# cbrl/BNN-PYNQ

Measured on AMD Instinct MI355X. Metric: images/sec (whole node) CNV-W1A1 CIFAR-10-shape batch, higher is better.
Workload: dtype u1; 1 GPU; cnvW1A1, 131072 synthetic 32x32x3 uint8 images per GPU per step, inputs resident in HBM, params cifar10/cnvW1A1; parallelism=dp1 (batch shards, no data-path collective)

## Files before the change

### bnn-pynq_amd/csrc/kernels.hip

```cpp
#include <hip/hip_runtime.h>
#include <hip/hip_ext.h>
#include <stdint.h>

#include <cstdlib>
#include <cstring>
#include <type_traits>

#define BNN_HD __host__ __device__
#include "act_faults.h"
#include "input_faults.h"
#include "kernels.h"
#include "mem_faults.h"
#include "mem_org.h"
#include "packed_params.h"
static_assert(bnn::kL0TileOffset == (int)bnn::kL0MfmaTileOffset && bnn::kL0BigBytes == (int)bnn::kL0MfmaBigBytes,
              "k_conv0_tile's operand offsets must be the ones packed_params.cpp writes the layer-0 table by");

namespace bnn {
namespace {

typedef const uint32_t __attribute__((address_space(4))) *kptr32;
typedef const uint64_t __attribute__((address_space(4))) *kptr64;

constexpr int kBlock = 256;
// ... 704 lines not shown
    for (int t0 = (wave / NT) * 32; t0 < nitems; t0 += 32 * STREAMS) {
      const int item = min(t0 + c, nitems - 1);
      const int i = item / IPI, rem = item - i * IPI, rp = rem / WOUT, x = rem - rp * WOUT;
      v16f acc[2] = {seed, seed};
#pragma unroll
      for (int kh = 0; kh < KH; kh++) {
        const uint4 *__restrict__ P = &plane[i][kh * 2 + h][2 * rp * WIN + x];
#pragma unroll
        for (int kx = 0; kx < 3; kx++) {
          v8i b[4];
#pragma unroll
          for (int y = 0; y < 4; y++) {
            const uint4 v = P[y * WIN + kx];
            b[y] = v8i{(int)v.x, (int)v.y, (int)v.z, (int)v.w, 0, 0, 0, 0};
          }
#pragma unroll
          for (int ky = 0; ky < 3; ky++)
#pragma unroll
            for (int dy = 0; dy < 2; dy++)
              acc[dy] = __builtin_amdgcn_mfma_scale_f32_32x32x64_f8f6f4(wreg[(ky * 3 + kx) * KH + kh], b[ky + dy], acc[dy], 4, 4, 0,
                                                                         0x7F7F7F7F, 0, 0x7F7F7F7F);
        }
      }
      const bool valid = t0 + c < nitems;
      const size_t img = (size_t)(img0 + i);
      if constexpr (POOL) {
        v16f top;
#pragma unroll
        for (int k = 0; k < 16; k++) top[k] = fmaxf(acc[0][k], acc[1][k]);
        uint32_t n0, n1;
        not_fired(top, dt, h, n0, n1);
        n0 &= (uint32_t)__builtin_amdgcn_mov_dpp((int)n0, 0xB1, 0xF, 0xF, true);
        n1 &= (uint32_t)__builtin_amdgcn_mov_dpp((int)n1, 0xB1, 0xF, 0xF, true);
        const size_t w64 = (img * (RP * RP) + rp * RP + (x >> 1)) * (NT / 2) + mt / 2;
        if (valid && !(x & 1)) out[(w64 * 2 + h) * 2 + (mt & 1)] = h ? ~(n0 ^ n1) : (n0 & n1);
      } else {
        uint32_t n0[2], n1[2];
#pragma unroll
        for (int dy = 0; dy < 2; dy++) not_fired(acc[dy], dt, h, n0[dy], n1[dy]);
        const uint32_t m0 = h ? n0[1] : n0[0], m1 = h ? n1[1] : n1[0];
        const size_t w64 = (img * (WOUT * WOUT) + (2 * rp + h) * WOUT + x) * (NT / 2) + mt / 2;
        if (valid) {
          out[(w64 * 2 + 0) * 2 + (mt & 1)] = m0 & m1;
          out[(w64 * 2 + 1) * 2 + (mt & 1)] = ~(m0 ^ m1);
        }
      }
    }
  }
}

template <bool TT>
__global__ __launch_bounds__(256) void k_conv_mfma_a2_table(const uint32_t *__restrict__ rows, int ksteps, int tiles,
                                                             uint8_t *__restrict__ dst) {
  const int idx = blockIdx.x * 256 + threadIdx.x, nw = ksteps * tiles * 64, row_dw = TT ? 4 + 6 * ksteps : 2 + 2 * ksteps;
  if (idx < nw) {
    const int ks = idx / (tiles * 64), mt = (idx / 64) % tiles, lane = idx & 63, n = 32 * mt + (lane & 31), h = lane >> 5;
    const uint32_t *__restrict__ row = rows + (size_t)n * row_dw;
    uint32_t b1, b2 = 0, b3;
    if constexpr (TT) {
      const uint32_t sg = row[2 + 4 * ks + h], two = row[2 + 4 * ksteps + 2 * ks + h], nz = row[2 + 4 * ks + 2 + h] | two;
      b1 = nz & ~two;
      b2 = two;
      b3 = (sg & nz) | two;
    } else {
      b1 = 0xFFFFFFFFu;
      b3 = row[2 + 2 * ks + h];
    }
    uint32_t v[4];
#pragma unroll
    for (int k = 0; k < 4; k++)
      v[k] = (nibble_spread(b1 >> (8 * k)) << 1) | (nibble_spread(b2 >> (8 * k)) << 2) | (nibble_spread(b3 >> (8 * k)) << 3);
    reinterpret_cast<uint4 *>(dst)[idx] = make_uint4(v[0], v[1], v[2], v[3]);
  } else if (idx < nw + tiles * 64) {
    const int j = idx - nw, second = j >= tiles * 32, jj = second ? j - tiles * 32 : j, mt = jj >> 5, h = (jj >> 4) & 1, reg = jj & 15;
    const int n = 32 * mt + (reg & 3) + 8 * (reg >> 2) + 4 * h;
    const int lim = 2 * 64 * ksteps;
    int t0 = (int)rows[(size_t)n * row_dw], t1 = (int)rows[(size_t)n * row_dw + 1];
    t0 = t0 < -lim - 1 ? -lim - 1 : (t0 > lim ? lim : t0);
    t1 = t1 < -lim - 1 ? -lim - 1 : (t1 > lim ? lim : t1);
    reinterpret_cast<float *>(dst + (size_t)nw * 16)[j] = second ? (float)(t1 - t0) : -(float)t0 - 0.5f;
  }
}

template <bool A2, int KS, int NT, bool CONV, int WAVES, int G>
__global__ __launch_bounds__(64 * WAVES, 8 / WAVES) void k_tail_mfma(const std::conditional_t<A2, uint4, uint32_t> *__restrict__ in,
                                                                      uint32_t *__restrict__ out, const uint8_t *__restrict__ tab,
                                                                      int n_images) {
  using U = std::conditional_t<A2, uint4, uint32_t>;
  constexpr int T = 64 * WAVES, TPW = NT / WAVES, IPI = CONV ? 9 : 1, W64 = CONV ? 25 * 2 : KS, UPI = A2 ? W64 : 2 * W64;
  constexpr int GP = G + 1, NPL = CONV ? G * 4 * 25 : 2 * KS * GP, NPF = (G * UPI + T - 1) / T, NC = (A2 ? 2 : 1) * NT * 2;
  static_assert(NT % WAVES == 0 && (!CONV || KS == 18) && (G * IPI) % 32 == 0, "tile geometry");
  __shared__ uint4 plane[NPL];
  __shared__ uint32_t lut[A2 ? 512 : 256];
  __shared__ v16f cst[NC];
  const int tid = threadIdx.x, lane = tid & 63, wave = tid >> 6, mt0 = wave * TPW, c = lane & 31, h = lane >> 5;
  for (int k = tid; k < 256; k += T) {
    if constexpr (A2) {
      lut[k] = nibble_spread((uint32_t)k) << 1;
      lut[256 + k] = nibble_spread((uint32_t)k) << 3;
    } else {
      lut[k] = fp4_pm1((uint32_t)k);
    }
  }
  for (int k = tid; k < NC * 16; k += T) reinterpret_cast<float *>(cst)[k] = reinterpret_cast<const float *>(tab + (size_t)KS * NT * 64 * 16)[k];
  const uint4 *__restrict__ wt = reinterpret_cast<const uint4 *>(tab);
  v8i wreg[TPW][KS];
#pragma unroll
  for (int j = 0; j < TPW; j++)
#pragma unroll
    for (int ks = 0; ks < KS; ks++) {
      const uint4 v = wt[(ks * NT + mt0 + j) * 64 + lane];
      wreg[j][ks] = v8i{(int)v.x, (int)v.y, (int)v.z, (int)v.w, 0, 0, 0, 0};
    }
  const int ngroups = (n_images + G - 1) / G;
  U pre[NPF];
  auto fetch = [&](int grp) {
    const int img0 = grp * G, lim = min(G, n_images - img0) * UPI;
#pragma unroll
    for (int j = 0; j < NPF; j++) {
      const int d = tid + T * j;
      pre[j] = d < lim ? in[(size_t)img0 * UPI + d] : U{};
    }
  };
  if (blockIdx.x < ngroups) fetch(blockIdx.x);
  for (int grp = blockIdx.x; grp < ngroups; grp += gridDim.x) {
    const int img0 = grp * G, nimg = min(G, n_images - img0), nitems = nimg * IPI;
    __syncthreads();
#pragma unroll
    for (int j = 0; j < NPF; j++) {
      const int d = tid + T * j;
      if (d < nimg * UPI) {
        const int i = d / UPI, e = d - i * UPI;
        if constexpr (A2) {
          const uint4 v = pre[j];
          const int p0 = CONV ? (i * 4 + 2 * (e & 1)) * 25 + (e >> 1) : 2 * e * GP + i, step = CONV ? 25 : GP;
          plane[p0] = fp4_planes(lut, lut + 256, v.x, v.z);
          plane[p0 + step] = fp4_planes(lut, lut + 256, v.y, v.w);
        } else {
          const uint32_t bits = pre[j];
          const int p0 = CONV ? (i * 4 + (e & 3)) * 25 + (e >> 2) : e * GP + i;
          plane[p0] = make_uint4(lut[bits & 255], lut[(bits >> 8) & 255], lut[(bits >> 16) & 255], lut[bits >> 24]);
        }
      }
    }
    if (grp + (int)gridDim.x < ngroups) fetch(grp + gridDim.x);
    __syncthreads();
#pragma clang loop unroll(disable) interleave(disable) vectorize(disable)
    for (int t0 = 0; t0 < nitems; t0 += 32) {
      const int item = min(t0 + c, nitems - 1);
      int base;
      if constexpr (CONV) {
        const int i = item / 9, p = item - i * 9, oy = p / 3, ox = p - oy * 3;
        base = (i * 4 + h) * 25 + oy * 5 + ox;
      } else {
        base = h * GP + item;
      }
      v16f acc[TPW];
#pragma unroll
      for (int j = 0; j < TPW; j++) acc[j] = cst[(mt0 + j) * 2 + h];
#pragma unroll
      for (int ks = 0; ks < KS; ks++) {
        const int off = CONV ? (ks & 1) * 2 * 25 + ((ks >> 1) / 3) * 5 + (ks >> 1) % 3 : ks * 2 * GP;
        const uint4 v = plane[base + off];
        const v8i b = v8i{(int)v.x, (int)v.y, (int)v.z, (int)v.w, 0, 0, 0, 0};
#pragma unroll
        for (int j = 0; j < TPW; j++)
          acc[j] = __builtin_amdgcn_mfma_scale_f32_32x32x64_f8f6f4(wreg[j][ks], b, acc[j], 4, 4, 0, 0x7F7F7F7F, 0, 0x7F7F7F7F);
      }
      const bool valid = t0 + c < nitems;
      const size_t gitem = (size_t)img0 * IPI + item;
#pragma unroll
      for (int j = 0; j < TPW; j++) {
        const int mt = mt0 + j;
        if constexpr (A2) {
          uint32_t n0, n1;
          not_fired(acc[j], cst[NT * 2 + mt * 2 + h], h, n0, n1);
          const size_t w64 = gitem * (NT / 2) + mt / 2;
          if (valid) out[(w64 * 2 + h) * 2 + (mt & 1)] = h ? ~(n0 ^ n1) : (n0 & n1);
        } else {
          int v[16];
#pragma unroll
          for (int k = 0; k < 16; k++) v[k] = __float_as_int(acc[j][k]);
          const uint32_t nf = or_halves(sign_nibbles(v, h));
          if (valid && h == (j & 1)) out[gitem * NT + mt] = ~nf;
        }
      }
    }
  }
}

__device__ __forceinline__ uint32_t chain_temp() {
  uint32_t t;
  asm("" : "=v"(t));
  return t;
}
#ifdef BNN_VGPR_COUNTER
#define SCALAR_COUNTER(c) do { } while (0)
#else
#define SCALAR_COUNTER(c) asm volatile("" : "+s"(c))
#endif
__device__ __forceinline__ void xpop(int &acc, uint32_t w, uint32_t a, uint32_t &t) {
  asm("v_xor_b32 %0, %2, %3\n\tv_bcnt_u32_b32 %1, %0, %1" : "+v"(t), "+v"(acc) : "s"(w), "v"(a));
}
__device__ __forceinline__ void xpop4(int &m0, int &m1, int &m2, int &m3, uint32_t w, uint32_t a0, uint32_t a1,
                                      uint32_t a2, uint32_t a3, uint32_t &t) {
  xpop(m0, w, a0, t); xpop(m1, w, a1, t); xpop(m2, w, a2, t); xpop(m3, w, a3, t);
}
__device__ __forceinline__ int xpop_seed(uint32_t w, uint32_t a, int seed, uint32_t &t) {
  int acc;
  asm("v_xor_b32 %0, %2, %3\n\tv_bcnt_u32_b32 %1, %0, %4" : "+v"(t), "=v"(acc) : "s"(w), "v"(a), "s"(seed));
  return acc;
}
template <int NPB>
__device__ __forceinline__ void store_group(uint32_t *__restrict__ out, size_t index, uint32_t bits) {
  if constexpr (NPB == 32) out[index] = bits;
  else reinterpret_cast<uint8_t *>(out)[index] = (uint8_t)bits;
}

template <int CW, int ID, bool POOL, int NPB = 32, bool MULTI = false>
__global__ __launch_bounds__(kBlock) void k_quad_x(const uint64_t *__restrict__ in, uint32_t *__restrict__ out,
                                                    const uint32_t *__restrict__ rows, int n_items, int groups, int gpb, MultiArgs ma = {}) {
  constexpr int OD = ID - 2, QD = OD / 2, NQ = QD * QD, KW = 9 * CW, ROW_DW = 2 + 2 * KW;
  int item0 = 0;
  if constexpr (MULTI) item0 = multi_prologue(ma, rows, out, n_items, 0);
  const BlockMap bm = map_block(groups / gpb, n_items);
  if (!bm.valid) return;
  const int item = bm.item + item0;
  const int img = item / NQ, q = item - img * NQ;
  const int qy = q / QD, qx = q - qy * QD;
  const uint64_t *__restrict__ base = in + ((size_t)img * ID * ID + (size_t)(2 * qy) * ID + 2 * qx) * CW;
  uint32_t wl[4][4][CW], wh[4][4][CW];
#pragma unroll
  for (int y = 0; y < 4; y++)
#pragma unroll
    for (int x = 0; x < 4; x++)
#pragma unroll
      for (int k = 0; k < CW; k++) {
        const uint64_t v = base[(y * ID + x) * CW + k];
        wl[y][x][k] = (uint32_t)v;
        wh[y][x][k] = (uint32_t)(v >> 32);
      }
  uint32_t t = chain_temp();
  for (int cg = bm.cg * gpb, cg_end = cg + gpb; cg < cg_end; cg++) {
    kptr32 w = (kptr32)(uintptr_t)(rows + (size_t)cg * NPB * ROW_DW);
    uint32_t b[4] = {0, 0, 0, 0};
    for (int c = NPB - 1; c >= 0; c--) {
      kptr32 r = w + c * ROW_DW;
      SCALAR_COUNTER(c);
      const int nt = -(int)r[0];
      int m[2][2];
  #pragma unroll
      for (int j = 0; j < KW; j++) {
        const int ky = j / (3 * CW), kx = (j / CW) % 3, k = j % CW;
        const uint32_t w0 = r[2 + 2 * j], w1 = r[3 + 2 * j];
        if (j == 0) {
  #pragma unroll
          for (int i = 0; i < 4; i++) m[i >> 1][i & 1] = xpop_seed(w0, wl[ky + (i >> 1)][kx + (i & 1)][k], nt, t);
        } else {
          xpop4(m[0][0], m[0][1], m[1][0], m[1][1], w0, wl[ky][kx][k], wl[ky][kx + 1][k], wl[ky + 1][kx][k], wl[ky + 1][kx + 1][k], t);
        }
        xpop4(m[0][0], m[0][1], m[1][0], m[1][1], w1, wh[ky][kx][k], wh[ky][kx + 1][k], wh[ky + 1][kx][k], wh[ky + 1][kx + 1][k], t);
      }
      if constexpr (POOL) {
        b[0] = shift_in_sign(b[0], min(min(m[0][0], m[0][1]), min(m[1][0], m[1][1])));
      } else {
  #pragma unroll
        for (int i = 0; i < 4; i++) b[i] = shift_in_sign(b[i], m[i >> 1][i & 1]);
      }
    }
// ... 502 lines not shown
  constexpr bool TWO = ARITH == AR_TT;
  constexpr int KW = 9 * CW, ROW_DW = row_dw<ARITH, KW>(), OD = ID - 2, NPIX = POOL ? (OD / 2) * (OD / 2) : OD * OD;
  const MultiSeg sg = multi_seg(ma);
  const int item0 = multi_prologue(ma, rows, out, n_items, 0);
  const BlockMap bm = map_block(groups / gpb, n_items);
  if (!bm.valid) return;
  const ActWinSite st = win_site(sites, sg.run);
  const WinItem wi = win_item<ID, POOL>(bm.item + item0, sg, st.y, st.x);
  const uint64_t *__restrict__ in = base + ((size_t)wi.image * ID * ID + (size_t)wi.oy * ID + wi.ox) * CW * 2;
  uint32_t as[KW][2], az[KW][2];
#pragma unroll
  for (int ky = 0; ky < 3; ky++)
#pragma unroll
    for (int kx = 0; kx < 3; kx++) {
      const bool hit = wi.oy + ky == st.y && wi.ox + kx == st.x;
#pragma unroll
      for (int k = 0; k < CW; k++) {
        const uint64_t *__restrict__ src = in + ((ky * ID + kx) * CW + k) * 2;
        uint64_t sgn = src[0], nz = src[1];
        if (hit && k == st.word) {
          const uint64_t m = 1ull << st.bit;
          const uint32_t i = (sgn & m) ? 0u : ((nz & m) ? 2u : 1u), lv = (i + (uint32_t)st.shift) % 3u;
          sgn = lv == 0 ? (sgn | m) : (sgn & ~m);
          nz = lv != 1 ? (nz | m) : (nz & ~m);
        }
        const int d = (ky * 3 + kx) * CW + k;
        as[d][0] = (uint32_t)sgn; as[d][1] = (uint32_t)(sgn >> 32);
        az[d][0] = (uint32_t)nz; az[d][1] = (uint32_t)(nz >> 32);
      }
    }
  int nn = 0;
  if constexpr (ARITH == AR_TB) {
#pragma unroll
    for (int k = 0; k < KW; k++) nn += __builtin_popcount(az[k][0]) + __builtin_popcount(az[k][1]);
  }
  uint32_t t = chain_temp();
  for (int cg = bm.cg * gpb, cg_end = cg + gpb; cg < cg_end; cg++) {
    kptr32 w = (kptr32)(uintptr_t)(rows + (size_t)cg * 32 * ROW_DW);
    uint32_t b0 = 0, b1 = 0;
    vec_group<ARITH, KW, true, 32, TWO>(w, as, az, nn, t, b0, b1);
    if constexpr (POOL) {
      b0 |= __shfl_xor(b0, 1, 64);
      b0 |= __shfl_xor(b0, 2, 64);
      b1 |= __shfl_xor(b1, 1, 64);
      b1 |= __shfl_xor(b1, 2, 64);
    }
    finish_bits<true>(b0, b1);
    if (wi.store) store_bits<true, 32>(out, (size_t)wi.slot * NPIX + wi.opix, groups, cg, b0, b1);
  }
}

template <int ARITH, int KW, bool TWO = false, bool MULTI = false>
__global__ __launch_bounds__(kBlock) void k_fclast(const uint64_t *__restrict__ in, int16_t *__restrict__ scores,
                                                    int32_t *__restrict__ classes, const uint32_t *__restrict__ rows,
                                                    int n_items, int number_class, MultiArgs ma = {}) {
  constexpr int PL = planes_in<ARITH>(), WPL = wplanes<ARITH>();
  constexpr int ROW_DW = row_dw<ARITH, KW>();
  if constexpr (MULTI) {
    const MultiSeg sg = multi_seg(ma);
    rows += (size_t)sg.run * ma.stride_dw;
    n_items = sg.len;
    in += (size_t)sg.slot * KW * PL;
    classes += (size_t)sg.run * ma.res_images + sg.image;
    scores = nullptr;
  }
  const int item = blockIdx.x * kBlock + threadIdx.x;
  if (item >= n_items) return;
  uint64_t as[KW], az[PL == 2 ? KW : 1];
  const uint64_t *__restrict__ base = in + (size_t)item * KW * PL;
#pragma unroll
  for (int k = 0; k < KW; k++) {
    as[k] = base[k * PL];
    if constexpr (PL == 2) az[k] = base[k * PL + 1];
  }
  int nzt = 0;
  if constexpr (ARITH == AR_TB) {
#pragma unroll
    for (int k = 0; k < KW; k++) nzt += pc64(az[k]);
  }
  kptr32 w = (kptr32)(uintptr_t)rows;
  uint32_t *__restrict__ s32 = reinterpret_cast<uint32_t *>(scores) + (size_t)item * 32;
  int best = 0, bestv = 0;
  uint32_t lo = 0;
  for (int n = 0; n < 64; n++) {
    kptr64 rw = (kptr64)(w + n * ROW_DW + 2);
    int m = 0, z = 0;
#pragma unroll
    for (int k = 0; k < KW; k++) mac<ARITH>(m, z, as[k], az[PL == 2 ? k : 0], rw + k * WPL);
    if constexpr (TWO) {
      if (w[n * ROW_DW + 2 + 6 * KW]) {
#pragma unroll
        for (int k = 0; k < KW; k++) z += two_extra64(rw[2 * KW + k], as[k], az[k]);
      }
    }
    int s = (ARITH == AR_XNOR) ? (KW * 64 - m) : finish<ARITH>(m, z, nzt);
    s = (int)(int16_t)s;
    if (n < number_class && s > bestv) { bestv = s; best = n; }
    if (scores) {
      if (n & 1) s32[n >> 1] = lo | ((uint32_t)(uint16_t)s << 16);
      else lo = (uint32_t)(uint16_t)s;
    }
  }
  if (classes) classes[item] = best;
}

template <int ARITH, int KW, bool TWO = false>
__global__ __launch_bounds__(kBlock) void k_fclast_wave(const uint64_t *__restrict__ in, int16_t *__restrict__ scores,
                                                         int32_t *__restrict__ classes, const uint32_t *__restrict__ rows,
                                                         int n_items, int number_class) {
  constexpr int PL = planes_in<ARITH>();
  constexpr int ROW_DW = row_dw<ARITH, KW>();
  const int lane = threadIdx.x & 63, item = blockIdx.x * (kBlock / 64) + (threadIdx.x >> 6);
  if (item >= n_items) return;
  const uint64_t *__restrict__ base = in + (size_t)item * KW * PL;
  const uint64_t *__restrict__ rw = reinterpret_cast<const uint64_t *>(rows + (size_t)lane * ROW_DW + 2);
  int m = 0, z = 0, nzt = 0;
#pragma unroll
  for (int k = 0; k < KW; k++) {
    const uint64_t as = base[k * PL], az = (PL == 2) ? base[k * PL + 1] : 0;
    if constexpr (ARITH == AR_XNOR) {
      m += pc64(rw[k] ^ as);
    } else if constexpr (ARITH == AR_TB) {
      m += pc64(az & (as ^ rw[k]));
      nzt += pc64(az);
    } else {
      const uint64_t zz = az & rw[k * 2 + 1];
      z += pc64(zz);
      m += pc64(zz & (as ^ rw[k * 2]));
    }
  }
  if constexpr (TWO) {
    if (rows[(size_t)lane * ROW_DW + 2 + 6 * KW]) {
#pragma unroll
      for (int k = 0; k < KW; k++) z += two_extra64(rw[2 * KW + k], base[k * PL], base[k * PL + 1]);
    }
  }
  int sc = (ARITH == AR_XNOR) ? (KW * 64 - m) : finish<ARITH>(m, z, nzt);
  sc = (int)(int16_t)sc;
  if (scores) scores[(size_t)item * 64 + lane] = (int16_t)sc;
  if (classes) {
    int key = (lane < number_class && sc > 0) ? sc * 64 + (63 - lane) : -1;
#pragma unroll
    for (int off = 32; off >= 1; off >>= 1) key = max(key, __shfl_xor(key, off, 64));
    if (lane == 0) classes[item] = key < 0 ? 0 : 63 - (key & 63);
  }
}

template <int KW>
__device__ __forceinline__ int xnor_row(const uint32_t *__restrict__ rows, int n, const uint64_t *act, int &thr) {
  constexpr int ROW_DW = 2 + 2 * KW;
  const uint32_t *__restrict__ r = rows + (size_t)n * ROW_DW;
  const uint64_t *__restrict__ w = reinterpret_cast<const uint64_t *>(r + 2);
  thr = (int)r[0];
  int m = 0;
#pragma unroll
  for (int k = 0; k < KW; k++) m += pc64(w[k] ^ act[k]);
  return m;
}

__global__ __launch_bounds__(512) void k_cnv_tail(const uint64_t *__restrict__ in, int16_t *__restrict__ scores,
                                                   int32_t *__restrict__ classes, const uint32_t *__restrict__ r4,
                                                   const uint32_t *__restrict__ r5, const uint32_t *__restrict__ r6,
                                                   const uint32_t *__restrict__ r7, const uint32_t *__restrict__ r8, int number_class,
                                                   unsigned *done, unsigned done_seq) {
  __shared__ uint64_t x3[50], x4[36], x5[4], x6[8], x7[8];
  const int t = threadIdx.x, lane = t & 63, wave = t >> 6, img = blockIdx.x;
  if (t < 50) x3[t] = in[(size_t)img * 50 + t];
// ... 985 lines not shown
      if (nthr == 1) row[1] = v;
    }
  }
  unsigned c = __popc(m);
#pragma unroll
  for (int d = 32; d >= 1; d >>= 1) {
    c += __shfl_xor(c, d, 64);
    phys += __shfl_xor(phys, d, 64);
  }
  if ((threadIdx.x & 63) == 0 && (phys | c)) {
    unsigned long long *const at = counts + (size_t)run * run_stride + (size_t)L.layer * 4 + 2;
    if (phys) atomicAdd(at, (unsigned long long)phys);
    if (c) atomicAdd(at + 1, (unsigned long long)c);
  }
}

inline long long lfc_fused_max() {
  static const long long v = [] {
    const char *e = std::getenv("BNN_MI355X_LFC_FUSED_MAX");
    return e ? std::atoll(e) : 1024LL;
  }();
  return v;
}
inline long long lfc_block_max() {
  static const long long v = [] {
    const char *e = std::getenv("BNN_MI355X_LFC_BLOCK_MAX");
    return e ? std::atoll(e) : 131072LL;
  }();
  return v;
}

inline long long l0_tile_min() {
  static const long long v = [] {
    const char *e = std::getenv("BNN_MI355X_L0_TILE_MIN");
    return e ? std::atoll(e) : 8192LL;
  }();
  return v;
}

constexpr long long kConvMfmaMinW1A2 = 384, kConvMfmaMinW2A2 = 256;
inline long long conv_mfma_min() {
  static const long long v = [] {
    const char *e = std::getenv("BNN_MI355X_CONV_MFMA_MIN");
    return e ? std::atoll(e) : 512LL;
  }();
  return v;
}
template <int ARITH>
inline long long conv_mfma_a2_min() {
  static const long long v = [] {
    const char *e = std::getenv("BNN_MI355X_CONV_MFMA_MIN");
    return e ? std::atoll(e) : (ARITH == AR_TT ? kConvMfmaMinW2A2 : kConvMfmaMinW1A2);
  }();
  return v;
}
template <int ARITH, bool OUT2>
inline const uint8_t *conv_mfma_for(const CnvLaunch &a) {
  if constexpr (ARITH == AR_XNOR && !OUT2) return a.n >= conv_mfma_min() ? a.conv_mfma : nullptr;
  else return a.n >= conv_mfma_a2_min<ARITH>() ? a.conv_mfma : nullptr;
}
constexpr long long kTailMfmaMinW1A1 = 3072, kTailMfmaMinW1A2 = 3072, kTailMfmaMinW2A2 = 1024;
constexpr int kTailMfmaStages = 0xF0;
template <int ARITH>
inline long long tail_mfma_min() {
  static const long long v = [] {
    const char *e = std::getenv("BNN_MI355X_TAIL_MFMA_MIN");
    return e ? std::atoll(e) : (ARITH == AR_XNOR ? kTailMfmaMinW1A1 : ARITH == AR_TB ? kTailMfmaMinW1A2 : kTailMfmaMinW2A2);
  }();
  return v;
}
template <int ARITH>
inline const uint8_t *tail_mfma_for(const CnvLaunch &a) {
  if (a.done_flag && a.n == 1) return nullptr;
  return a.n >= tail_mfma_min<ARITH>() ? a.conv_mfma : nullptr;
}
inline unsigned persistent_grid(long long units, long long cap) {
  const long long per = (units + cap - 1) / cap;
  return (unsigned)((units + per - 1) / per);
}
constexpr long long kConvMfmaGrid = 512;
constexpr int kConvMfmaImgsL1 = 2, kConvMfmaImgs = 8;
constexpr int kTailMfmaImgsL4 = 32, kTailMfmaImgsL5 = 32, kTailMfmaImgsFc = 128;
constexpr long long kTailMfmaGrid8 = 256;
#define BNN_TAIL_MFMA(A2, KS, NT, CONV, WAVES, G, cap, in, out, tab)                                                               \
  hipLaunchKernelGGL((k_tail_mfma<A2, KS, NT, CONV, WAVES, G>), dim3(persistent_grid((n + (G) - 1) / (G), (cap))), dim3(64 * (WAVES)), 0, s, \
                     in, out, tab, (int)n)

inline int gpb_for(long long items, int groups) { return (items + kBlock - 1) / kBlock >= 2048 ? groups : 1; }

inline bool narrow_for(long long items, int groups32, long long limit) { return ((items + kBlock - 1) / kBlock) * groups32 < limit; }
constexpr long long kNarrowLimitCnv = 8192, kNarrowLimitLfc = 512;
constexpr long long kFcLastWaveMax = 32768;
constexpr long long kPixelLaneMax = 512;
constexpr long long kCnvTailMax = 1024;

inline dim3 grid_for(long long items, int groups) {
  const long long item_blocks = (items + kBlock - 1) / kBlock;
  return dim3((unsigned)(((item_blocks + 7) / 8) * 8 * groups));
}

#define BNN_LAUNCH(kern, grid, stream, ...)                                   \
  do {                                                                        \
    if ((grid).x > 0) hipLaunchKernelGGL(kern, grid, dim3(kBlock), 0, stream, __VA_ARGS__); \
  } while (0)
#define BNN_STAGE(kern32, kern8, items, groups32, in, out, rows)                                                                   \
  do {                                                                                                                             \
    const long long it_ = (items);                                                                                                 \
    if (narrow_for(it_, (groups32), narrow_limit)) BNN_LAUNCH(kern8, grid_for(it_, (groups32) * 4), s, in, out, rows, (int)it_, (groups32) * 4, 1); \
    else BNN_LAUNCH(kern32, grid_for(it_, (groups32) / gpb_for(it_, (groups32))), s, in, out, rows, (int)it_, (groups32), gpb_for(it_, (groups32))); \
  } while (0)
#define BNN_MARK(ev, i, stream)                          \
  do {                                                   \
    if (ev) (void)hipEventRecord((ev)[i], stream);       \
  } while (0)

template <int ARITH, bool OUT2, bool TWO = false>
void run_cnv_t(const CnvLaunch &a) {
  const long long n = a.n, narrow_limit = kNarrowLimitCnv;
  uint32_t *A = reinterpret_cast<uint32_t *>(a.buf0), *B = reinterpret_cast<uint32_t *>(a.buf1);
  const uint64_t *A64 = reinterpret_cast<const uint64_t *>(a.buf0), *B64 = reinterpret_cast<const uint64_t *>(a.buf1);
  hipStream_t s = a.stream;
  BNN_MARK(a.events, 0, s);
  if (a.l0_mfma) {
    const dim3 g0((unsigned)((n * 900 + kBlock - 1) / kBlock));
    if (a.last_stage >= 0) {
      if (n >= l0_tile_min()) BNN_LAUNCH((k_conv0_tile<OUT2>), dim3((unsigned)((n + kL0Imgs - 1) / kL0Imgs)), s, a.images, A, a.l0_mfma, (int)n);
      else BNN_LAUNCH((k_conv0_mfma<OUT2>), g0, s, a.images, A, a.l0_mfma, (int)(n * 900));
    }
  } else {
    if (a.last_stage >= 0) BNN_LAUNCH((k_conv0<OUT2>), grid_for(n * 900, 2 / gpb_for(n * 900, 2)), s, a.images, A, a.rows[0], (int)(n * 900), 2, gpb_for(n * 900, 2));
  }
  BNN_MARK(a.events, 1, s);
  if constexpr (ARITH == AR_XNOR && !OUT2) {
    const bool pix = n <= kPixelLaneMax;
    const uint8_t *const cm = conv_mfma_for<ARITH, OUT2>(a);
    const dim3 g1(persistent_grid((n + kConvMfmaImgsL1 - 1) / kConvMfmaImgsL1, kConvMfmaGrid)),
        gm(persistent_grid((n + kConvMfmaImgs - 1) / kConvMfmaImgs, kConvMfmaGrid));
    if (a.last_stage >= 1) {
      if (a.l1_literal) {
        BNN_LAUNCH(k_l1_literal, dim3((unsigned)((n * 784 + kBlock - 1) / kBlock)), s, A64, reinterpret_cast<uint64_t *>(B), a.rows[1], (int)(n * 784));
      } else if (a.l1_mfma) {
        const long long pairs = (n + 1) / 2;
        hipLaunchKernelGGL(k_l1_mfma, dim3((unsigned)(pairs < 512 ? pairs : 512)), dim3(256), 0, s, reinterpret_cast<const uint32_t *>(a.buf0), B,
                           a.l1_mfma, (int)n);
      } else if (cm) {
        hipLaunchKernelGGL((k_conv_mfma<30, 2, 2, true, kConvMfmaImgsL1>), g1, dim3(256), 0, s, reinterpret_cast<const uint32_t *>(a.buf0), B, cm,
                           (int)n);
      } else if (pix) BNN_LAUNCH((k_vec_x<9, true, 1, 30, 8, true>), grid_for(n * 784, 8), s, A64, B, a.rows[1], (int)(n * 784), 8, 1);
      else BNN_STAGE((k_quad_x<1, 30, true>), (k_quad_x<1, 30, true, 8>), n * 196, 2, A64, B, a.rows[1]);
    }
    BNN_MARK(a.events, 2, s);
    if (a.last_stage >= 2) {
      if (cm) hipLaunchKernelGGL((k_conv_mfma<14, 2, 4, false, kConvMfmaImgs>), gm, dim3(256), 0, s, B, A, cm + kConvMfmaL2Off, (int)n);
      else if (pix) BNN_LAUNCH((k_vec_x<9, true, 1, 14, 8>), grid_for(n * 144, 16), s, B64, A, a.rows[2], (int)(n * 144), 16, 1);
      else BNN_STAGE((k_quad_x<1, 14, false>), (k_quad_x<1, 14, false, 8>), n * 36, 4, B64, A, a.rows[2]);
    }
    BNN_MARK(a.events, 3, s);
    if (a.last_stage >= 3) {
      if (cm) hipLaunchKernelGGL((k_conv_mfma<12, 4, 4, true, kConvMfmaImgs>), gm, dim3(256), 0, s, A, B, cm + kConvMfmaL3Off, (int)n);
      else if (pix) BNN_LAUNCH((k_vec_x<18, true, 2, 12, 8, true>), grid_for(n * 100, 16), s, A64, B, a.rows[3], (int)(n * 100), 16, 1);
      else BNN_STAGE((k_quad_x<2, 12, true>), (k_quad_x<2, 12, true, 8>), n * 25, 4, A64, B, a.rows[3]);
    }
    BNN_MARK(a.events, 4, s);
    const uint8_t *const tm = tail_mfma_for<ARITH>(a);
    const uint32_t *const A32 = A, *const B32 = B;
    if (!tm && n <= kCnvTailMax && !a.events && a.last_stage >= kCnvStages - 1) {
      hipLaunchKernelGGL(k_cnv_tail, dim3((unsigned)n), dim3(512), 0, s, B64, a.scores, a.classes, a.rows[4], a.rows[5], a.rows[6],
                         a.rows[7], a.rows[8], a.number_class, n == 1 ? a.done_flag : nullptr, a.done_seq);
      return;
    }
    if (a.last_stage >= 4) {
      if (tm && (kTailMfmaStages & 16)) BNN_TAIL_MFMA(false, 18, 8, true, 8, kTailMfmaImgsL4, kTailMfmaGrid8, B32, A, tm + kTailMfmaL4Off);
      else BNN_STAGE((k_vec_x<18, true, 2, 5>), (k_vec_x<18, true, 2, 5, 8>), n * 9, 8, B64, A, a.rows[4]);
    }
    BNN_MARK(a.events, 5, s);
    if (a.last_stage >= 5) {
      if (tm && (kTailMfmaStages & 32)) BNN_TAIL_MFMA(false, 36, 8, false, 8, kTailMfmaImgsL5, kTailMfmaGrid8, A32, B, tm + kTailMfmaL5Off);
      else BNN_STAGE((k_vec_x<36, false, 1, 1>), (k_vec_x<36, false, 1, 1, 8>), n, 8, A64, B, a.rows[5]);
    }
    BNN_MARK(a.events, 6, s);
    if (a.last_stage >= 6) {
      if (tm && (kTailMfmaStages & 64)) BNN_TAIL_MFMA(false, 4, 16, false, 4, kTailMfmaImgsFc, kConvMfmaGrid, B32, A, tm + kTailMfmaL6Off);
      else BNN_STAGE((k_vec_x<4, false, 1, 1>), (k_vec_x<4, false, 1, 1, 8>), n, 16, B64, A, a.rows[6]);
    }
    BNN_MARK(a.events, 7, s);
    if (a.last_stage >= 7) {
      if (tm && (kTailMfmaStages & 128)) BNN_TAIL_MFMA(false, 8, 16, false, 8, kTailMfmaImgsFc, kTailMfmaGrid8, A32, B, tm + kTailMfmaL7Off);
      else BNN_STAGE((k_vec_x<8, false, 1, 1>), (k_vec_x<8, false, 1, 1, 8>), n, 16, A64, B, a.rows[7]);
    }
    BNN_MARK(a.events, 8, s);
  } else {
    const bool pix = n <= kPixelLaneMax;
    const uint8_t *const cm = conv_mfma_for<ARITH, OUT2>(a);
    const uint4 *const A128 = reinterpret_cast<const uint4 *>(a.buf0), *const B128 = reinterpret_cast<const uint4 *>(a.buf1);
    const dim3 g1(persistent_grid((n + kConvMfmaImgsL1 - 1) / kConvMfmaImgsL1, kConvMfmaGrid)),
        gm(persistent_grid((n + kConvMfmaImgs - 1) / kConvMfmaImgs, kConvMfmaGrid));
    if (a.last_stage >= 1) {
      if (cm) hipLaunchKernelGGL((k_conv_mfma_a2<30, 2, 2, true, kConvMfmaImgsL1>), g1, dim3(256), 0, s, A128, B, cm, (int)n);
      else if (pix) BNN_LAUNCH((k_vec<ARITH, 9, OUT2, true, 1, 30, 8, true, TWO>), grid_for(n * 784, 8), s, A64, B, a.rows[1], (int)(n * 784), 8, 1);
      else BNN_STAGE((k_quad<ARITH, 1, 30, true, OUT2, 32, TWO>), (k_quad<ARITH, 1, 30, true, OUT2, 8, TWO>), n * 196, 2, A64, B, a.rows[1]);
    }
    BNN_MARK(a.events, 2, s);
    if (a.last_stage >= 2) {
      if (cm) hipLaunchKernelGGL((k_conv_mfma_a2<14, 2, 4, false, kConvMfmaImgs>), gm, dim3(256), 0, s, B128, A, cm + kConvMfmaA2L2Off, (int)n);
      else if (pix) BNN_LAUNCH((k_vec<ARITH, 9, OUT2, true, 1, 14, 8, false, TWO>), grid_for(n * 144, 16), s, B64, A, a.rows[2], (int)(n * 144), 16, 1);
      else BNN_STAGE((k_quad<ARITH, 1, 14, false, OUT2, 32, TWO>), (k_quad<ARITH, 1, 14, false, OUT2, 8, TWO>), n * 36, 4, B64, A, a.rows[2]);
    }
    BNN_MARK(a.events, 3, s);
    if (a.last_stage >= 3) {
      if (cm) hipLaunchKernelGGL((k_conv_mfma_a2<12, 4, 4, true, kConvMfmaImgs>), gm, dim3(256), 0, s, A128, B, cm + kConvMfmaA2L3Off, (int)n);
      else if (pix) BNN_LAUNCH((k_vec<ARITH, 18, OUT2, true, 2, 12, 8, true, TWO>), grid_for(n * 100, 16), s, A64, B, a.rows[3], (int)(n * 100), 16, 1);
      else BNN_STAGE((k_quad<ARITH, 2, 12, true, OUT2, 32, TWO>), (k_quad<ARITH, 2, 12, true, OUT2, 8, TWO>), n * 25, 4, A64, B, a.rows[3]);
    }
    BNN_MARK(a.events, 4, s);
    const uint8_t *const tm = tail_mfma_for<ARITH>(a);
    if constexpr (!TWO) {
      if (!tm && n <= kCnvTailMax && !a.events && a.last_stage >= kCnvStages - 1) {
        hipLaunchKernelGGL((k_cnv_tail_a2<ARITH>), dim3((unsigned)n), dim3(512), 0, s, B64, a.scores, a.classes, a.rows[4], a.rows[5],
                           a.rows[6], a.rows[7], a.rows[8], a.number_class, n == 1 ? a.done_flag : nullptr, a.done_seq);
        return;
      }
    }
    if (a.last_stage >= 4) {
      if (tm && (kTailMfmaStages & 16)) BNN_TAIL_MFMA(true, 18, 8, true, 8, kTailMfmaImgsL4, kTailMfmaGrid8, B128, A, tm + kTailMfmaA2L4Off);
      else BNN_STAGE((k_vec<ARITH, 18, OUT2, true, 2, 5, 32, false, TWO>), (k_vec<ARITH, 18, OUT2, true, 2, 5, 8, false, TWO>), n * 9, 8, B64, A, a.rows[4]);
    }
    BNN_MARK(a.events, 5, s);
    if (a.last_stage >= 5) {
      if (tm && (kTailMfmaStages & 32)) BNN_TAIL_MFMA(true, 36, 8, false, 8, kTailMfmaImgsL5, kTailMfmaGrid8, A128, B, tm + kTailMfmaA2L5Off);
      else BNN_STAGE((k_vec<ARITH, 36, OUT2, false, 1, 1, 32, false, TWO>), (k_vec<ARITH, 36, OUT2, false, 1, 1, 8, false, TWO>), n, 8, A64, B, a.rows[5]);
    }
    BNN_MARK(a.events, 6, s);
    if (a.last_stage >= 6) {
      if (tm && (kTailMfmaStages & 64)) BNN_TAIL_MFMA(true, 4, 16, false, 4, kTailMfmaImgsFc, kConvMfmaGrid, B128, A, tm + kTailMfmaA2L6Off);
      else BNN_STAGE((k_vec<ARITH, 4, OUT2, false, 1, 1, 32, false, TWO>), (k_vec<ARITH, 4, OUT2, false, 1, 1, 8, false, TWO>), n, 16, B64, A, a.rows[6]);
    }
    BNN_MARK(a.events, 7, s);
    if (a.last_stage >= 7) {
      if (tm && (kTailMfmaStages & 128)) BNN_TAIL_MFMA(true, 8, 16, false, 8, kTailMfmaImgsFc, kTailMfmaGrid8, A128, B, tm + kTailMfmaA2L7Off);
      else BNN_STAGE((k_vec<ARITH, 8, OUT2, false, 1, 1, 32, false, TWO>), (k_vec<ARITH, 8, OUT2, false, 1, 1, 8, false, TWO>), n, 16, A64, B, a.rows[7]);
    }
    BNN_MARK(a.events, 8, s);
  }
  if (a.last_stage >= 8) {
    if (n <= kFcLastWaveMax) BNN_LAUNCH((k_fclast_wave<ARITH, 8, TWO>), dim3((unsigned)((n + 3) / 4)), s, B64, a.scores, a.classes, a.rows[8], (int)n, a.number_class);
    else BNN_LAUNCH((k_fclast<ARITH, 8, TWO>), grid_for(n, 1), s, B64, a.scores, a.classes, a.rows[8], (int)n, a.number_class);
  }
  BNN_MARK(a.events, 9, s);
}

template <int ARITH, bool OUT2>
int matrix_stages_t(const CnvLaunch &a) {
  const bool cm = conv_mfma_for<ARITH, OUT2>(a) != nullptr;
  bool l1 = cm;
  if constexpr (ARITH == AR_XNOR && !OUT2) l1 = !a.l1_literal && (a.l1_mfma || cm);
  return (a.l0_mfma ? 1 : 0) | (l1 ? 2 : 0) | (cm ? 12 : 0) | (tail_mfma_for<ARITH>(a) ? kTailMfmaStages : 0);
}

#define BNN_MULTI(kern, ipi, groups32, in, out, rows, RES)                                                               \
  do {                                                                                                                   \
    const long long it_ = (long long)a.total * (ipi);                                                                    \
    const int gpb_ = gpb_for(it_, (groups32));                                                                           \
    const MultiArgs ma_{a.segs, (unsigned)(a.stride / 4), (ipi), (RES) ? a.n : 0};                                       \
// ... 488 lines not shown
```

Before: 40.56 million images/s.

## Fuse FC6/FC7/classifier into one MFMA kernel and pipeline single-tile tail loads

Result: no change. 40.92 million images/s, median of 6 (+0.9%).

```diff
diff --git a/bnn-pynq_amd/csrc/kernels.hip b/bnn-pynq_amd/csrc/kernels.hip
--- a/bnn-pynq_amd/csrc/kernels.hip
+++ b/bnn-pynq_amd/csrc/kernels.hip
@@ -810,6 +810,11 @@
   }
 }
 
+#ifdef BNN_TAIL_MFMA_AHEAD
+constexpr int kTailMfmaAhead = BNN_TAIL_MFMA_AHEAD;
+#else
+constexpr int kTailMfmaAhead = 3;
+#endif
 template <bool A2, int KS, int NT, bool CONV, int WAVES, int G>
 __global__ __launch_bounds__(64 * WAVES, 8 / WAVES) void k_tail_mfma(const std::conditional_t<A2, uint4, uint32_t> *__restrict__ in,
                                                                       uint32_t *__restrict__ out, const uint8_t *__restrict__ tab,
@@ -820,7 +825,7 @@
   static_assert(NT % WAVES == 0 && (!CONV || KS == 18) && (G * IPI) % 32 == 0, "tile geometry");
   __shared__ uint4 plane[NPL];
   __shared__ uint32_t lut[A2 ? 512 : 256];
-  __shared__ v16f cst[NC];
+  __shared__ v16f cst[TPW > 1 ? NC : 1];
   const int tid = threadIdx.x, lane = tid & 63, wave = tid >> 6, mt0 = wave * TPW, c = lane & 31, h = lane >> 5;
   for (int k = tid; k < 256; k += T) {
     if constexpr (A2) {
@@ -830,7 +835,8 @@
       lut[k] = fp4_pm1((uint32_t)k);
     }
   }
-  for (int k = tid; k < NC * 16; k += T) reinterpret_cast<float *>(cst)[k] = reinterpret_cast<const float *>(tab + (size_t)KS * NT * 64 * 16)[k];
+  if constexpr (TPW > 1)
+    for (int k = tid; k < NC * 16; k += T) reinterpret_cast<float *>(cst)[k] = reinterpret_cast<const float *>(tab + (size_t)KS * NT * 64 * 16)[k];
   const uint4 *__restrict__ wt = reinterpret_cast<const uint4 *>(tab);
   v8i wreg[TPW][KS];
 #pragma unroll
@@ -840,6 +846,13 @@
       const uint4 v = wt[(ks * NT + mt0 + j) * 64 + lane];
       wreg[j][ks] = v8i{(int)v.x, (int)v.y, (int)v.z, (int)v.w, 0, 0, 0, 0};
     }
+  [[maybe_unused]] v16f seed, dt;
+  if constexpr (TPW == 1) {
+    const v16f *__restrict__ ct = reinterpret_cast<const v16f *>(tab + (size_t)KS * NT * 64 * 16);
+    seed = ct[mt0 * 2 + h];
+    if constexpr (A2) dt = ct[NT * 2 + mt0 * 2 + h];
+    __builtin_amdgcn_s_waitcnt(0x0F70);
+  }
   const int ngroups = (n_images + G - 1) / G;
   U pre[NPF];
   auto fetch = [&](int grp) {
@@ -850,6 +863,7 @@
       pre[j] = d < lim ? in[(size_t)img0 * UPI + d] : U{};
     }
   };
+  [[maybe_unused]] const int ci0 = c / 9, cp0 = c - ci0 * 9;
   if (blockIdx.x < ngroups) fetch(blockIdx.x);
   for (int grp = blockIdx.x; grp < ngroups; grp += gridDim.x) {
     const int img0 = grp * G, nimg = min(G, n_images - img0), nitems = nimg * IPI;
@@ -873,27 +887,53 @@
     }
     if (grp + (int)gridDim.x < ngroups) fetch(grp + gridDim.x);
     __syncthreads();
+    [[maybe_unused]] int ci = ci0, cp = cp0;
 #pragma clang loop unroll(disable) interleave(disable) vectorize(disable)
     for (int t0 = 0; t0 < nitems; t0 += 32) {
-      const int item = min(t0 + c, nitems - 1);
+      const int item = TPW == 1 ? t0 + c : min(t0 + c, nitems - 1);
       int base;
-      if constexpr (CONV) {
+      if constexpr (CONV && TPW == 1) {
+        base = (ci * 4 + h) * 25 + cp + 2 * ((cp * 11) >> 5);
+      } else if constexpr (CONV) {
         const int i = item / 9, p = item - i * 9, oy = p / 3, ox = p - oy * 3;
         base = (i * 4 + h) * 25 + oy * 5 + ox;
       } else {
         base = h * GP + item;
       }
-      v16f acc[TPW];
-#pragma unroll
-      for (int j = 0; j < TPW; j++) acc[j] = cst[(mt0 + j) * 2 + h];
-#pragma unroll
-      for (int ks = 0; ks < KS; ks++) {
+      auto read = [&](v8i &b, int ks) {
         const int off = CONV ? (ks & 1) * 2 * 25 + ((ks >> 1) / 3) * 5 + (ks >> 1) % 3 : ks * 2 * GP;
         const uint4 v = plane[base + off];
-        const v8i b = v8i{(int)v.x, (int)v.y, (int)v.z, (int)v.w, 0, 0, 0, 0};
-#pragma unroll
-        for (int j = 0; j < TPW; j++)
-          acc[j] = __builtin_amdgcn_mfma_scale_f32_32x32x64_f8f6f4(wreg[j][ks], b, acc[j], 4, 4, 0, 0x7F7F7F7F, 0, 0x7F7F7F7F);
+        b = v8i{(int)v.x, (int)v.y, (int)v.z, (int)v.w, 0, 0, 0, 0};
+      };
+      v16f acc[TPW];
+      if constexpr (TPW == 1) {
+        constexpr int D = kTailMfmaAhead;
+        v8i b[D + 1];
+#pragma unroll
+        for (int ks = 0; ks < D; ks++) read(b[ks], ks);
+        acc[0] = seed;
+#pragma unroll
+        for (int ks = 0; ks < KS; ks++) {
+          __builtin_amdgcn_sched_barrier(0);
+          acc[0] = __builtin_amdgcn_mfma_scale_f32_32x32x64_f8f6f4(wreg[0][ks], b[ks % (D + 1)], acc[0], 4, 4, 0, 0x7F7F7F7F, 0, 0x7F7F7F7F);
+          if (ks + D < KS) read(b[(ks + D) % (D + 1)], ks + D);
+        }
+        __builtin_amdgcn_sched_barrier(0);
+        if constexpr (CONV) {
+          ci += 3, cp += 5;
+          if (cp >= 9) cp -= 9, ci += 1;
+        }
+      } else {
+#pragma unroll
+        for (int j = 0; j < TPW; j++) acc[j] = cst[(mt0 + j) * 2 + h];
+#pragma unroll
+        for (int ks = 0; ks < KS; ks++) {
+          v8i b;
+          read(b, ks);
+#pragma unroll
+          for (int j = 0; j < TPW; j++)
+            acc[j] = __builtin_amdgcn_mfma_scale_f32_32x32x64_f8f6f4(wreg[j][ks], b, acc[j], 4, 4, 0, 0x7F7F7F7F, 0, 0x7F7F7F7F);
+        }
       }
       const bool valid = t0 + c < nitems;
       const size_t gitem = (size_t)img0 * IPI + item;
@@ -902,7 +942,8 @@
         const int mt = mt0 + j;
         if constexpr (A2) {
           uint32_t n0, n1;
-          not_fired(acc[j], cst[NT * 2 + mt * 2 + h], h, n0, n1);
+          if constexpr (TPW == 1) not_fired(acc[j], dt, h, n0, n1);
+          else not_fired(acc[j], cst[NT * 2 + mt * 2 + h], h, n0, n1);
           const size_t w64 = gitem * (NT / 2) + mt / 2;
           if (valid) out[(w64 * 2 + h) * 2 + (mt & 1)] = h ? ~(n0 ^ n1) : (n0 & n1);
         } else {
@@ -913,6 +954,124 @@
           if (valid && h == (j & 1)) out[gitem * NT + mt] = ~nf;
         }
       }
+    }
+  }
+}
+
+template <int G>
+__global__ __launch_bounds__(512, 1) void k_fc_mfma(const uint32_t *__restrict__ in, int32_t *__restrict__ classes,
+                                                     const uint8_t *__restrict__ tab6, const uint8_t *__restrict__ tab7,
+                                                     const uint32_t *__restrict__ rows8, int n_images, int number_class) {
+  constexpr int T = 512, K6 = 4, K7 = 8, NT = 16, GP = G + 1, GX = G + 4, NPF = G * 8 / T, ROW8 = 2 + 2 * 8;
+  static_assert(G % 32 == 0 && (G * 8) % T == 0, "whole item tiles, whole expansion passes");
+  __shared__ uint4 p6[2 * K6 * GP], p7[2 * K7 * GP];
+  __shared__ uint32_t x7[NT * GX];
+  __shared__ uint32_t lut[256];
+  __shared__ v16f cst[2 * NT * 2];
+  __shared__ uint4 w8[64 * 4];
+  const int tid = threadIdx.x, lane = tid & 63, wave = tid >> 6, mt0 = wave * 2, c = lane & 31, h = lane >> 5;
+  for (int k = tid; k < 256; k += T) lut[k] = fp4_pm1((uint32_t)k);
+  for (int k = tid; k < NT * 32; k += T) {
+    reinterpret_cast<float *>(cst)[k] = reinterpret_cast<const float *>(tab6 + (size_t)K6 * NT * 64 * 16)[k];
+    reinterpret_cast<float *>(cst)[NT * 32 + k] = reinterpret_cast<const float *>(tab7 + (size_t)K7 * NT * 64 * 16)[k];
+  }
+  for (int k = tid; k < 64 * 16; k += T) reinterpret_cast<uint32_t *>(w8)[k] = rows8[(k >> 4) * ROW8 + 2 + (k & 15)];
+  v8i w6[2][K6], w7[2][K7];
+#pragma unroll
+  for (int j = 0; j < 2; j++) {
+#pragma unroll
+    for (int ks = 0; ks < K6; ks++) {
+      const uint4 v = reinterpret_cast<const uint4 *>(tab6)[(ks * NT + mt0 + j) * 64 + lane];
+      w6[j][ks] = v8i{(int)v.x, (int)v.y, (int)v.z, (int)v.w, 0, 0, 0, 0};
+    }
+#pragma unroll
+    for (int ks = 0; ks < K7; ks++) {
+      const uint4 v = reinterpret_cast<const uint4 *>(tab7)[(ks * NT + mt0 + j) * 64 + lane];
+      w7[j][ks] = v8i{(int)v.x, (int)v.y, (int)v.z, (int)v.w, 0, 0, 0, 0};
+    }
+  }
+  auto expand = [&](uint32_t bits) { return make_uint4(lut[bits & 255], lut[(bits >> 8) & 255], lut[(bits >> 16) & 255], lut[bits >> 24]); };
+  auto word = [&](const v16f &acc) {
+    int v[16];
+#pragma unroll
+    for (int k = 0; k < 16; k++) v[k] = __float_as_int(acc[k]);
+    return ~or_halves(sign_nibbles(v, h));
+  };
+  const int ngroups = (n_images + G - 1) / G, nrows = min(number_class, 64);
+  uint32_t pre[NPF];
+  auto fetch = [&](int grp) {
+    const int img0 = grp * G, lim = min(G, n_images - img0) * 8;
+#pragma unroll
+    for (int j = 0; j < NPF; j++) {
+      const int d = tid + T * j;
+      pre[j] = d < lim ? in[(size_t)img0 * 8 + d] : 0u;
+    }
+  };
+  if (blockIdx.x < ngroups) fetch(blockIdx.x);
+  __syncthreads();
+  for (int grp = blockIdx.x; grp < ngroups; grp += gridDim.x) {
+    const int img0 = grp * G, nimg = min(G, n_images - img0);
+    uint32_t cur[NPF];
+#pragma unroll
+    for (int j = 0; j < NPF; j++) cur[j] = pre[j];
+    if (grp + (int)gridDim.x < ngroups) fetch(grp + gridDim.x);
+#pragma unroll
+    for (int j = 0; j < NPF; j++) {
+      const int d = tid + T * j;
+      p6[(d & 7) * GP + (d >> 3)] = expand(cur[j]);
+    }
+    __syncthreads();
+#pragma clang loop unroll(disable) interleave(disable) vectorize(disable)
+    for (int t0 = 0; t0 < nimg; t0 += 32) {
+      v16f acc[2] = {cst[mt0 * 2 + h], cst[(mt0 + 1) * 2 + h]};
+#pragma unroll
+      for (int ks = 0; ks < K6; ks++) {
+        const uint4 v = p6[(2 * ks + h) * GP + t0 + c];
+        const v8i b = v8i{(int)v.x, (int)v.y, (int)v.z, (int)v.w, 0, 0, 0, 0};
+#pragma unroll
+        for (int j = 0; j < 2; j++)
+          acc[j] = __builtin_amdgcn_mfma_scale_f32_32x32x64_f8f6f4(w6[j][ks], b, acc[j], 4, 4, 0, 0x7F7F7F7F, 0, 0x7F7F7F7F);
+      }
+#pragma unroll
+      for (int j = 0; j < 2; j++) {
+        const uint4 e = expand(word(acc[j]));
+        if (h == j) p7[(mt0 + j) * GP + t0 + c] = e;
+      }
+    }
+    __syncthreads();
+#pragma clang loop unroll(disable) interleave(disable) vectorize(disable)
+    for (int t0 = 0; t0 < nimg; t0 += 32) {
+      v16f acc[2] = {cst[NT * 2 + mt0 * 2 + h], cst[NT * 2 + (mt0 + 1) * 2 + h]};
+#pragma unroll
+      for (int ks = 0; ks < K7; ks++) {
+        const uint4 v = p7[(2 * ks + h) * GP + t0 + c];
+        const v8i b = v8i{(int)v.x, (int)v.y, (int)v.z, (int)v.w, 0, 0, 0, 0};
+#pragma unroll
+        for (int j = 0; j < 2; j++)
+          acc[j] = __builtin_amdgcn_mfma_scale_f32_32x32x64_f8f6f4(w7[j][ks], b, acc[j], 4, 4, 0, 0x7F7F7F7F, 0, 0x7F7F7F7F);
+      }
+#pragma unroll
+      for (int j = 0; j < 2; j++) {
+        const uint32_t bits = word(acc[j]);
+        if (h == j) x7[(mt0 + j) * GX + t0 + c] = bits;
+      }
+    }
+    __syncthreads();
+    for (int il = tid >> 2; il < nimg; il += T / 4) {
+      const int q = tid & 3;
+      uint32_t a[4];
+#pragma unroll
+      for (int k = 0; k < 4; k++) a[k] = x7[(4 * q + k) * GX + il];
+      int best = 0, bestv = 0;
+      for (int n = 0; n < nrows; n++) {
+        const uint4 w = w8[n * 4 + q];
+        int m = __builtin_popcount(w.x ^ a[0]) + __builtin_popcount(w.y ^ a[1]) + __builtin_popcount(w.z ^ a[2]) + __builtin_popcount(w.w ^ a[3]);
+        m += __builtin_amdgcn_mov_dpp(m, 0xB1, 0xF, 0xF, true);
+        m += __builtin_amdgcn_mov_dpp(m, 0x4E, 0xF, 0xF, true);
+        const int s = (int)(int16_t)(8 * 64 - m);
+        if (s > bestv) { bestv = s; best = n; }
+      }
+      if (q == 0) classes[(size_t)img0 + il] = best;
     }
   }
 }
@@ -1581,7 +1740,8 @@
   uint32_t *__restrict__ s32 = reinterpret_cast<uint32_t *>(scores) + (size_t)item * 32;
   int best = 0, bestv = 0;
   uint32_t lo = 0;
-  for (int n = 0; n < 64; n++) {
+  const int nrows = scores ? 64 : min(number_class, 64);
+  for (int n = 0; n < nrows; n++) {
     kptr64 rw = (kptr64)(w + n * ROW_DW + 2);
     int m = 0, z = 0;
 #pragma unroll
@@ -2733,6 +2893,18 @@
 constexpr int kConvMfmaImgsL1 = 2, kConvMfmaImgs = 8;
 constexpr int kTailMfmaImgsL4 = 32, kTailMfmaImgsL5 = 32, kTailMfmaImgsFc = 128;
 constexpr long long kTailMfmaGrid8 = 256;
+#ifdef BNN_FC_MFMA_IMGS
+constexpr int kFcMfmaImgs = BNN_FC_MFMA_IMGS;
+#else
+constexpr int kFcMfmaImgs = 128;
+#endif
+inline bool fc_fused_on() {
+  static const bool on = [] {
+    const char *e = std::getenv("BNN_MI355X_FC_FUSED");
+    return !(e && std::atoi(e) == 0);
+  }();
+  return on;
+}
 #define BNN_TAIL_MFMA(A2, KS, NT, CONV, WAVES, G, cap, in, out, tab)                                                               \
   hipLaunchKernelGGL((k_tail_mfma<A2, KS, NT, CONV, WAVES, G>), dim3(persistent_grid((n + (G) - 1) / (G), (cap))), dim3(64 * (WAVES)), 0, s, \
                      in, out, tab, (int)n)
@@ -2830,6 +3002,11 @@
       else BNN_STAGE((k_vec_x<36, false, 1, 1>), (k_vec_x<36, false, 1, 1, 8>), n, 8, A64, B, a.rows[5]);
     }
     BNN_MARK(a.events, 6, s);
+    if (tm && (kTailMfmaStages & 192) == 192 && fc_fused_on() && !a.events && a.last_stage >= kCnvStages - 1 && !a.scores && a.classes) {
+      hipLaunchKernelGGL((k_fc_mfma<kFcMfmaImgs>), dim3(persistent_grid((n + kFcMfmaImgs - 1) / kFcMfmaImgs, kTailMfmaGrid8)), dim3(512), 0, s, B32,
+                         a.classes, tm + kTailMfmaL6Off, tm + kTailMfmaL7Off, a.rows[8], (int)n, a.number_class);
+      return;
+    }
     if (a.last_stage >= 6) {
       if (tm && (kTailMfmaStages & 64)) BNN_TAIL_MFMA(false, 4, 16, false, 4, kTailMfmaImgsFc, kConvMfmaGrid, B32, A, tm + kTailMfmaL6Off);
       else BNN_STAGE((k_vec_x<4, false, 1, 1>), (k_vec_x<4, false, 1, 1, 8>), n, 16, B64, A, a.rows[6]);
```
